# lizhe00/AnimatableGaussians

Hardware: AMD Instinct MI355X
Metric: rendered views/sec (fwd+bwd) @1024^2, ~250k Gaussians (higher is better)
Workload: dtype f32; 1 GPU; BASELINE configs[1]: avatar front|back map, 1 view @1024x1024 per step, rasterizer fwd+bwd through the library-owned step (ag_raster_forward_backward, one native call per view; per-camera argument structures and output images prepared once, FusedRasterStep.prepare / run); gaussians=268348, tiles=4096, views=8, streams=3, prewarm=300, parallelism=1 process

## Files before the change

animatablegaussians_amd/_lib.py:

```python
from __future__ import annotations

import ctypes
import os

import torch

_HERE = os.path.dirname(os.path.abspath(__file__))
LIB_PATH = os.environ.get("AG_LIB_PATH") or os.path.join(_HERE, "lib", "libag_hip.so")

c_i32 = ctypes.c_int32
c_f = ctypes.c_float
c_vp = ctypes.c_void_p
c_sz = ctypes.c_size_t


class AgRasterForwardArgs(ctypes.Structure):
    _fields_ = [
        ("P", c_i32), ("W", c_i32), ("H", c_i32),
        ("sh_degree", c_i32), ("sh_coeffs", c_i32), ("prefiltered", c_i32),
        ("tan_fovx", c_f), ("tan_fovy", c_f), ("scale_modifier", c_f),
        ("bg", c_vp), ("means3D", c_vp), ("colors_precomp", c_vp), ("shs", c_vp), ("opacities", c_vp),
        ("scales", c_vp), ("rotations", c_vp), ("cov3D_precomp", c_vp),
        ("viewmatrix", c_vp), ("projmatrix", c_vp), ("campos", c_vp),
        ("out_color", c_vp), ("out_depth", c_vp), ("out_alpha", c_vp), ("radii", c_vp),
# ... 5 lines not shown

class AgRasterBackwardArgs(ctypes.Structure):
    _fields_ = [
        ("P", c_i32), ("W", c_i32), ("H", c_i32),
        ("sh_degree", c_i32), ("sh_coeffs", c_i32), ("num_rendered", c_i32),
        ("tan_fovx", c_f), ("tan_fovy", c_f), ("scale_modifier", c_f),
        ("bg", c_vp), ("means3D", c_vp), ("radii", c_vp), ("colors_precomp", c_vp), ("shs", c_vp),
        ("scales", c_vp), ("rotations", c_vp), ("cov3D_precomp", c_vp),
        ("viewmatrix", c_vp), ("projmatrix", c_vp), ("campos", c_vp), ("alphas", c_vp),
        ("dL_dout_color", c_vp), ("dL_dout_depth", c_vp), ("dL_dout_alpha", c_vp),
        ("geom_buffer", c_vp), ("image_buffer", c_vp), ("binning_buffer", c_vp),
        ("dL_dmeans2D", c_vp), ("dL_dcolors", c_vp), ("dL_dopacity", c_vp), ("dL_dmeans3D", c_vp),
        ("dL_dcov3D", c_vp), ("dL_dsh", c_vp), ("dL_dscales", c_vp), ("dL_drotations", c_vp),
        ("accum_buffer", c_vp), ("accum_bytes", c_sz), ("accumulate", c_i32), ("reserved", c_i32),
    ]


class AgRasterScratchLayout(ctypes.Structure):
    _fields_ = [(n, c_sz) for n in (
        "geom_rec_off", "geom_rec_stride", "geom_cov3d_off", "geom_tiles_touched_off",
        "img_ranges_off", "img_n_contrib_off", "img_tile_count_off", "img_num_rendered_off",
        "bin_point_list_off", "bin_keys_off")]


class AgGatherArgs(ctypes.Structure):
    _fields_ = [("N", c_i32), ("S", c_i32)] + [(n, c_vp) for n in (
        "pix", "position_map", "other_map", "color_map", "xyz", "opacity_raw", "scaling_raw", "rotation_raw",
        "positions", "opacity", "scales", "rotations", "colors")]


# ... 94 lines not shown
    ("ag_last_error", ctypes.c_char_p, []),
    ("ag_raster_geom_bytes", c_sz, [c_i32]),
    ("ag_raster_image_bytes", c_sz, [c_i32, c_i32]),
    ("ag_raster_binning_bytes", c_sz, [c_i32]),
    ("ag_raster_accum_bytes", c_sz, [c_i32]),
    ("ag_raster_describe_scratch", ctypes.c_int, [c_i32, c_i32, c_i32, c_i32, ctypes.POINTER(AgRasterScratchLayout)]),
    ("ag_raster_forward_plan", ctypes.c_int, [ctypes.POINTER(AgRasterForwardArgs), c_vp, ctypes.POINTER(c_i32)]),
    ("ag_raster_forward_render", ctypes.c_int, [ctypes.POINTER(AgRasterForwardArgs), c_i32, c_vp]),
    ("ag_raster_forward_optimistic", ctypes.c_int, [ctypes.POINTER(AgRasterForwardArgs), c_i32, c_vp, ctypes.POINTER(c_i32)]),
    ("ag_raster_backward", ctypes.c_int, [ctypes.POINTER(AgRasterBackwardArgs), c_vp]),
    ("ag_raster_forward_backward", ctypes.c_int, [ctypes.POINTER(AgRasterForwardArgs), ctypes.POINTER(AgRasterBackwardArgs), c_i32, c_vp,
                                                  ctypes.POINTER(c_i32)]),
    ("ag_raster_forward_backward_enqueue", ctypes.c_int, [ctypes.POINTER(AgRasterForwardArgs), ctypes.POINTER(AgRasterBackwardArgs), c_i32, c_vp,
                                                          ctypes.POINTER(c_i32)]),
    ("ag_raster_collect", ctypes.c_int, [c_i32, ctypes.POINTER(c_i32)]),
    ("ag_raster_large_tile_sort", ctypes.c_int, [c_i32]),
    ("ag_raster_mark_visible", ctypes.c_int, [c_i32, c_vp, c_vp, c_vp, c_vp, c_vp]),
    ("ag_prof_kernel_name", ctypes.c_char_p, [c_i32]),
    ("ag_prof_enable", ctypes.c_int, [ctypes.c_uint32]),
    ("ag_prof_collect", ctypes.c_int, [ctypes.POINTER(c_i32), ctypes.POINTER(c_f), ctypes.POINTER(ctypes.c_double)]),
    ("ag_prof_collect_to", ctypes.c_int, [ctypes.c_char_p, ctypes.POINTER(c_i32), ctypes.POINTER(c_f), ctypes.POINTER(ctypes.c_double)]),
    ("ag_debug_atomic_rate", ctypes.c_int, [c_vp, c_i32, c_i32, c_i32, c_i32, c_vp]),
    ("ag_noise_bias_act_forward", ctypes.c_int, [c_vp, c_vp, c_vp, c_vp, c_vp, ctypes.c_int32, ctypes.c_int32, ctypes.c_float,
                                               ctypes.c_float, c_vp]),
    ("ag_noise_bias_act_partial_floats", c_sz, [c_i32, c_i32]),
    ("ag_noise_bias_act_backward", ctypes.c_int, [c_vp, c_vp, c_vp, c_vp, c_vp, c_vp, c_vp, ctypes.c_int32, ctypes.c_int32,
                                                ctypes.c_float, ctypes.c_float, c_vp]),
    ("ag_modulate_weight_forward", ctypes.c_int, [c_vp, c_vp, c_vp, c_vp, ctypes.c_float, ctypes.c_int32, ctypes.c_int32,
                                                ctypes.c_int32, ctypes.c_int32, ctypes.c_int32, c_vp]),
    ("ag_modulate_weight_partial_floats", c_sz, [c_i32, c_i32]),
# ... 173 lines not shown
```

animatablegaussians_amd/csrc/ag_abi.hip:

```cpp
#include <atomic>
#include <cstdarg>
#include <cstdio>
#include <mutex>
#include <cstring>
#include <vector>

#include "ag_common.h"

namespace ag {

static thread_local char g_err[512] = "";

void set_error(const char* fmt, ...)
{
    va_list ap;
    va_start(ap, fmt);
    vsnprintf(g_err, sizeof(g_err), fmt, ap);
    va_end(ap);
}

int check_hip(hipError_t e, const char* what)
{
    if (e == hipSuccess) return AG_OK;
    set_error("%s: %s", what, hipGetErrorString(e));
// ... 139 lines not shown
    return AG_OK;
}

int ag_raster_forward_optimistic(const AgRasterForwardArgs* a, int32_t capacity, void* stream, int32_t* num_rendered_host)
{
    if (!num_rendered_host) { set_error("null num_rendered_host"); return AG_ERR_INVALID_ARGUMENT; }
    *num_rendered_host = 0;
    if (capacity <= 0) { set_error("capacity must be positive"); return AG_ERR_INVALID_ARGUMENT; }
    int rc = validate_forward(a, true, capacity);
    if (rc) return rc;
    if (a->P == 0) return ag_raster_forward_render(a, 0, stream);
    hipStream_t s = reinterpret_cast<hipStream_t>(stream);
    int32_t* w = pinned_word();
    hipEvent_t ev = plan_event();
    if (!w || !ev) { set_error("hipHostMalloc / hipEventCreate failed"); return AG_ERR_HIP; }
    const bool skip_large = g_large_tiles_seen.load(std::memory_order_relaxed) == 0;
    if ((rc = launch_preprocess(*a, s))) return rc;
    if ((rc = launch_tile_scan(*a, s, (uint32_t)capacity, skip_large))) return rc;
    ImageLayout il((size_t)a->W, (size_t)a->H);
    const char* ib = aligned_base(a->image_buffer);
    if ((rc = check_hip(hipMemcpyAsync(w, ib + il.num_rendered, 4 * sizeof(int32_t), hipMemcpyDeviceToHost, s), "read num_rendered"))) return rc;
    if ((rc = check_hip(hipEventRecord(ev, s), "record plan event"))) return rc;
    if ((rc = launch_bin_sort(*a, capacity, s, skip_large))) return rc;
    if ((rc = launch_blend_forward(*a, capacity, s))) return rc;
    if ((rc = check_hip(hipEventSynchronize(ev), "wait for the instance count"))) return rc;
    *num_rendered_host = w[0];
    if (w[3] > 0) g_large_tiles_seen.store(1, std::memory_order_relaxed);
    if (w[2]) {
        if (w[0] <= capacity) set_error("optimistic forward: %d tiles of >= 2048 instances and the large-class sort was not enqueued for this frame; redo it", w[3]);
        else set_error("optimistic forward: %d instances exceed the capacity of %d; redo with ag_raster_forward_plan + _render", w[0], capacity);
        return AG_ERR_SCRATCH_TOO_SMALL;
    }
    return AG_OK;
}

int ag_raster_forward_render(const AgRasterForwardArgs* a, int32_t R, void* stream)
{
    int rc = validate_forward(a, true, R);
// ... 65 lines not shown
            if (pass == 0 && t.dev != dev) continue;
            if (pass == 1 && t.dev != -1) continue;
            if (t.dev == -1) {
                if (hipHostMalloc(reinterpret_cast<void**>(&t.w), 64, hipHostMallocDefault) != hipSuccess) { t.w = nullptr; return -1; }
                if (hipEventCreateWithFlags(&t.ev, hipEventDisableTiming) != hipSuccess) { (void)hipHostFree(t.w); t.w = nullptr; t.ev = nullptr; return -1; }
                t.dev = dev;
            }
            t.busy = true; t.capacity = capacity;
            return i;
        }
    return -1;
}
}

int ag_raster_forward_backward_enqueue(const AgRasterForwardArgs* f, AgRasterBackwardArgs* b, int32_t capacity, void* stream, int32_t* ticket)
{
    if (!f || !b || !ticket) { set_error("null args"); return AG_ERR_INVALID_ARGUMENT; }
    *ticket = -1;
    if (capacity <= 0) { set_error("capacity must be positive"); return AG_ERR_INVALID_ARGUMENT; }
    if (f->shs && !f->colors_precomp) { set_error("ag_raster_forward_backward: colours-precomp path only"); return AG_ERR_UNSUPPORTED; }
    b->P = f->P; b->W = f->W; b->H = f->H; b->sh_degree = f->sh_degree; b->sh_coeffs = f->sh_coeffs; b->num_rendered = capacity;
    b->tan_fovx = f->tan_fovx; b->tan_fovy = f->tan_fovy; b->scale_modifier = f->scale_modifier;
    b->bg = f->bg; b->means3D = f->means3D; b->radii = f->radii; b->colors_precomp = f->colors_precomp; b->shs = f->shs;
    b->scales = f->scales; b->rotations = f->rotations; b->cov3D_precomp = f->cov3D_precomp;
    b->viewmatrix = f->viewmatrix; b->projmatrix = f->projmatrix; b->campos = f->campos; b->alphas = f->out_alpha;
    b->geom_buffer = f->geom_buffer; b->image_buffer = f->image_buffer; b->binning_buffer = f->binning_buffer;
    int rc = validate_forward(f, true, capacity);
    if (rc) return rc;
    if ((rc = validate_backward(b))) return rc;
    if (f->P == 0) return ag_raster_forward_render(f, 0, stream);
    hipStream_t s = reinterpret_cast<hipStream_t>(stream);
    const int tk = ticket_acquire(capacity);
    if (tk < 0) { set_error("no free read-back ticket (64 views pending) or hipHostMalloc / hipEventCreate failed"); return AG_ERR_HIP; }
    Ticket& t = g_tk[tk];
    auto fail = [&](int code) { std::lock_guard<std::mutex> lk(g_tk_mu); t.busy = false; return code; };
    const bool skip_large = g_large_tiles_seen.load(std::memory_order_relaxed) == 0;
    if ((rc = launch_preprocess(*f, s))) return fail(rc);
    if ((rc = launch_tile_scan(*f, s, (uint32_t)capacity, skip_large))) return fail(rc);
    ImageLayout il((size_t)f->W, (size_t)f->H);
    const char* ib = aligned_base(f->image_buffer);
    if ((rc = check_hip(hipMemcpyAsync(t.w, ib + il.num_rendered, 4 * sizeof(int32_t), hipMemcpyDeviceToHost, s), "read num_rendered"))) return fail(rc);
    if ((rc = check_hip(hipEventRecord(t.ev, s), "record plan event"))) return fail(rc);
    if ((rc = launch_bin_sort(*f, capacity, s, skip_large))) return fail(rc);
    if ((rc = launch_blend_forward(*f, capacity, s))) return fail(rc);
    if ((rc = launch_blend_backward(*b, s))) return fail(rc);
    if ((rc = launch_preprocess_backward(*b, s))) return fail(rc);
    *ticket = tk;
    return AG_OK;
}

int ag_raster_collect(int32_t ticket, int32_t* num_rendered_host)
{
    if (!num_rendered_host) { set_error("null num_rendered_host"); return AG_ERR_INVALID_ARGUMENT; }
    *num_rendered_host = 0;
    if (ticket < 0 || ticket >= kTickets || !g_tk[ticket].busy) { set_error("ag_raster_collect: no such pending view (%d)", ticket); return AG_ERR_INVALID_ARGUMENT; }
    Ticket& t = g_tk[ticket];
    const int rc = check_hip(hipEventSynchronize(t.ev), "wait for the instance count");
    const int32_t n = t.w[0], over = t.w[2], n_large = t.w[3], cap = t.capacity;
    { std::lock_guard<std::mutex> lk(g_tk_mu); t.busy = false; }
    if (rc) return rc;
    *num_rendered_host = n;
    if (n_large > 0) g_large_tiles_seen.store(1, std::memory_order_relaxed);
    if (over) {
        if (n <= cap) set_error("forward+backward: %d tiles of >= 2048 instances and the large-class sort was not enqueued for this view; redo it", n_large);
        else set_error("forward+backward: %d instances exceed the capacity of %d; redo the view with a larger capacity", n, cap);
        return AG_ERR_SCRATCH_TOO_SMALL;
    }
    return AG_OK;
}

int ag_raster_large_tile_sort(int32_t mode)
{
    if (mode == 0 || mode == 1) g_large_tiles_seen.store(mode, std::memory_order_relaxed);
    else if (mode != -1) { set_error("ag_raster_large_tile_sort: mode must be -1 (query), 0 or 1"); return AG_ERR_INVALID_ARGUMENT; }
    return g_large_tiles_seen.load(std::memory_order_relaxed);
}

int ag_raster_forward_backward(const AgRasterForwardArgs* f, AgRasterBackwardArgs* b, int32_t capacity, void* stream,
                               int32_t* num_rendered_host)
// ... 81 lines not shown
```

animatablegaussians_amd/csrc/ag_binning.hip:

```cpp
#include <mutex>

#include "ag_common.h"

namespace ag {

__global__ void __launch_bounds__(1024) tile_scan_kernel(int T, const uint32_t* __restrict__ tile_count,
                                                        uint32_t* __restrict__ cursor, uint2* __restrict__ ranges,
                                                        uint32_t* __restrict__ num_rendered,
                                                        uint4* __restrict__ tile_order, uint32_t capacity, uint32_t skip_large)
{
    __shared__ uint32_t wave_sums[16], wave_ne[16];
    __shared__ uint32_t carry_s, carry_ne;
    __shared__ uint32_t cls_hist[34], cls_off[34];
    const int tid = threadIdx.x, lane = tid & 63, wave = tid >> 6;
    if (tid == 0) { carry_s = 0; carry_ne = 0; }
    if (tid < 34) cls_hist[tid] = 0;
    __syncthreads();
    const uint4* count4 = reinterpret_cast<const uint4*>(tile_count);
    const bool one_pass = T <= 4096;
    uint32_t keep_c[4] = {0u, 0u, 0u, 0u}, keep_st[4] = {0u, 0u, 0u, 0u};
    for (int base = 0; base < T; base += 4096) {
        const int t0 = base + 4 * tid;
        uint32_t c[4] = {0u, 0u, 0u, 0u};
        if (t0 + 3 < T) {
            const uint4 v4 = count4[t0 >> 2];
            c[0] = v4.x; c[1] = v4.y; c[2] = v4.z; c[3] = v4.w;
        } else {
#pragma unroll
            for (int k = 0; k < 4; k++) if (t0 + k < T) c[k] = tile_count[t0 + k];
        }
// ... 21 lines not shown
            r4[0] = make_uint4(c[0] ? start[0] : 0u, c[0] ? start[1] : 0u, c[1] ? start[1] : 0u, c[1] ? start[2] : 0u);
            r4[1] = make_uint4(c[2] ? start[2] : 0u, c[2] ? start[3] : 0u, c[3] ? start[3] : 0u, c[3] ? start[4] : 0u);
        } else {
#pragma unroll
            for (int k = 0; k < 4; k++)
                if (t0 + k < T) {
                    cursor[t0 + k] = start[k];
                    ranges[t0 + k] = c[k] ? make_uint2(start[k], start[k + 1]) : make_uint2(0u, 0u);
                }
        }
#pragma unroll
        for (int k = 0; k < 4; k++)
            if (t0 + k < T) {
                if (c[k]) {
                    atomicAdd(&cls_hist[32 - __clz(c[k])], 1u);
                    ne_before++;
                } else {
                    tile_order[(uint32_t)(T - 1) - ((uint32_t)(t0 + k) - ne_before)] = make_uint4((uint32_t)(t0 + k), 0u, 0u, 0u);
                }
            }
#pragma unroll
        for (int k = 0; k < 4; k++) { keep_c[k] = c[k]; keep_st[k] = start[k]; }
        __syncthreads();
        if (tid == 1023) { carry_s = start[4]; carry_ne = ne_before; }
        __syncthreads();
    }
    if (tid == 0) {
        uint32_t n_large = 0;
        for (int cls = 12; cls < 34; cls++) n_large += cls_hist[cls];
        const bool over = carry_s > capacity || (skip_large && n_large > 0u);
        num_rendered[0] = carry_s;
        num_rendered[1] = over ? 0u : carry_ne;
        num_rendered[2] = over ? 1u : 0u;
        num_rendered[3] = n_large;
    }
    if (tid == 0) {
        uint32_t acc = 0;
        for (int cls = 33; cls >= 1; cls--) { cls_off[cls] = acc; acc += cls_hist[cls]; }
    }
    __syncthreads();
    for (int base = 0; base < T; base += 4096) {
        const int t0 = base + 4 * tid;
        if (t0 >= T) break;
        uint32_t c[4] = {0u, 0u, 0u, 0u}, st[4] = {0u, 0u, 0u, 0u};
        if (one_pass) {
#pragma unroll
            for (int k = 0; k < 4; k++) { c[k] = keep_c[k]; st[k] = keep_st[k]; }
        } else if (t0 + 3 < T) {
            const uint4 v4 = count4[t0 >> 2], s4 = reinterpret_cast<const uint4*>(cursor)[t0 >> 2];
            c[0] = v4.x; c[1] = v4.y; c[2] = v4.z; c[3] = v4.w;
            st[0] = s4.x; st[1] = s4.y; st[2] = s4.z; st[3] = s4.w;
        } else {
#pragma unroll
            for (int k = 0; k < 4; k++) if (t0 + k < T) { c[k] = tile_count[t0 + k]; st[k] = cursor[t0 + k]; }
        }
#pragma unroll
        for (int k = 0; k < 4; k++)
            if (t0 + k < T) {
                if (c[k]) tile_order[atomicAdd(&cls_off[32 - __clz(c[k])], 1u)] = make_uint4((uint32_t)(t0 + k), st[k], st[k] + c[k], 0u);
            }
    }
}

int launch_tile_scan(const AgRasterForwardArgs& a, hipStream_t s, uint32_t capacity, bool skip_large)
{
    const int gx = (a.W + kTileX - 1) / kTileX, gy = (a.H + kTileY - 1) / kTileY;
    char* ib = aligned_base(a.image_buffer);
    ImageLayout il((size_t)a.W, (size_t)a.H);
    { ProfScope ps(AG_K_TILE_SCAN, s); hipLaunchKernelGGL(tile_scan_kernel, dim3(1), dim3(1024), 0, s, gx * gy,
                       reinterpret_cast<const uint32_t*>(ib + il.tile_count),
                       reinterpret_cast<uint32_t*>(ib + il.cursor),
                       reinterpret_cast<uint2*>(ib + il.ranges),
                       reinterpret_cast<uint32_t*>(ib + il.num_rendered),
                       reinterpret_cast<uint4*>(ib + il.tile_order), capacity, skip_large ? 1u : 0u); }
    return check_hip(hipGetLastError(), "tile_scan_kernel");
}

__device__ __forceinline__ void get_rect_i(float px, float py, int max_radius, int gx, int gy,
                                           uint32_t& x0o, uint32_t& y0o, uint32_t& x1o, uint32_t& y1o)
{
    const float r = (float)max_radius;
    int x0 = (int)((px - r) / (float)kTileX);
    int y0 = (int)((py - r) / (float)kTileY);
    int x1 = (int)((px + r + (float)kTileX - 1.0f) / (float)kTileX);
    int y1 = (int)((py + r + (float)kTileY - 1.0f) / (float)kTileY);
    x0 = max(0, x0); y0 = max(0, y0); x1 = max(0, x1); y1 = max(0, y1);
    x0o = (uint32_t)min(gx, x0); y0o = (uint32_t)min(gy, y0);
    x1o = (uint32_t)min(gx, x1); y1o = (uint32_t)min(gy, y1);
}
// ... 153 lines not shown
            const uint32_t blk = t >> lk, off = t & (hk - 1);
            const uint32_t i = (blk << (lk + 1)) + off, p = (blk << (lk + 1)) + k - 1 - off;
            if (p < n) { const uint64_t a = sk[i], b = sk[p]; if (a > b) { sk[i] = b; sk[p] = a; } }
        }
        __syncthreads();
        for (uint32_t j = k >> 2; j > 0; j >>= 1) {
            for (uint32_t t = tid; t < half; t += nthreads) {
                const uint32_t i = ((t & ~(j - 1)) << 1) | (t & (j - 1)), p = i + j;
                if (p < n) { const uint64_t a = sk[i], b = sk[p]; if (a > b) { sk[i] = b; sk[p] = a; } }
            }
            __syncthreads();
        }
    }
}

template <int NT, int KPT, bool PRESORTED>
__device__ __forceinline__ void sort_segment_lds(uint64_t* __restrict__ sk, const uint64_t* __restrict__ seg, uint32_t n, uint32_t run0,
                                                 uint32_t* __restrict__ out_list, uint64_t* __restrict__ out_keys, int tid)
{
    constexpr uint32_t CAP = NT * KPT;
    uint64_t* bufA = sk;
    uint64_t* bufB = sk + CAP;
    uint64_t v[KPT];
    const uint32_t base = (uint32_t)tid * (uint32_t)KPT;
#pragma unroll
    for (int i = 0; i < KPT; i++) v[i] = (base + i < n) ? seg[base + i] : kKeyInf;
    constexpr bool WAVE_RUNS = !PRESORTED && KPT == 4 && AG_SORT_WAVE_NETWORK;
    if constexpr (WAVE_RUNS) {
        if constexpr (KPT == 4) wave_sort256(v, tid & 63);
    } else if (!PRESORTED) sort_regs<KPT>(v);
    if (base < n) {
#pragma unroll
        for (int i = 0; i < KPT; i++) bufA[base + i] = v[i];
    }
    __syncthreads();
    const uint32_t n8 = (n + (uint32_t)KPT - 1u) & ~((uint32_t)KPT - 1u);
    for (uint32_t L = PRESORTED ? run0 : (WAVE_RUNS ? 256u : (uint32_t)KPT); L < n8; L <<= 1) {
        if (base < n8) {
            const uint32_t ps = base & ~(2u * L - 1u);
            const uint32_t o = base - ps;
            const uint32_t lx = min(L, n8 - ps);
            const uint32_t ly = (ps + L < n8) ? min(L, n8 - ps - L) : 0u;
            const uint64_t* X = bufA + ps;
            const uint64_t* Y = bufA + ps + L;
            uint32_t lo = (o > ly) ? o - ly : 0u, hi = min(o, lx);
            while (lo < hi) {
                const uint32_t mid = (lo + hi) >> 1;
                if (X[mid] < Y[o - mid - 1]) lo = mid + 1; else hi = mid;
            }
            uint32_t i = lo, j = o - lo;
            uint64_t xv = (i < lx) ? X[i] : kKeyInf, yv = (j < ly) ? Y[j] : kKeyInf;
#pragma unroll
            for (int r = 0; r < KPT; r++) {
                const bool takex = xv <= yv;
                bufB[base + r] = takex ? xv : yv;
                if (takex) { i++; xv = (i < lx) ? X[i] : kKeyInf; }
                else       { j++; yv = (j < ly) ? Y[j] : kKeyInf; }
            }
        }
        __syncthreads();
        uint64_t* t = bufA; bufA = bufB; bufB = t;
    }
    if (out_list) { for (uint32_t i = tid; i < n; i += NT) out_list[i] = (uint32_t)bufA[i]; }
    else          { for (uint32_t i = tid; i < n; i += NT) out_keys[i] = bufA[i]; }
}

template <int NT, bool LARGE, int KPT>
__global__ void __launch_bounds__(NT) tile_sort_kernel(const uint4* __restrict__ tile_order, const uint32_t* __restrict__ counts,
                                                      uint64_t* __restrict__ keys, uint32_t* __restrict__ point_list)
{
    extern __shared__ __attribute__((aligned(16))) uint64_t sk[];
    constexpr uint32_t CAP = NT * KPT;
    const uint32_t n_active = counts[1];
    const int tid = threadIdx.x;
    if (!LARGE) {
        for (uint32_t item = gridDim.x - 1u - blockIdx.x; item < 4u * n_active; item += gridDim.x) {
            const uint4 wd = tile_order[item >> 2];
            const uint32_t n = wd.z - wd.y;
            if (n < 2048u) break;
            if (n <= (uint32_t)kSortSmallCap || n > (uint32_t)kSortLargeCap) continue;
            const uint32_t c0 = (item & 3u) * (uint32_t)kSortSmallCap;
            if (c0 >= n) continue;
            __syncthreads();
            uint64_t* seg = keys + wd.y + c0;
            sort_segment_lds<NT, KPT, false>(sk, seg, min((uint32_t)kSortSmallCap, n - c0), 0u, nullptr, seg, tid);
        }
    }
    for (uint32_t rank = blockIdx.x; rank < n_active; rank += gridDim.x) {
    const uint4 wd = tile_order[rank];
    const uint2 rg = make_uint2(wd.y, wd.z);
    const uint32_t n = rg.y - rg.x;
    if (LARGE) { if (n < 2048u) break; if (n <= (uint32_t)kSortSmallCap) continue; }
    else if (n > (uint32_t)kSortSmallCap) continue;
    uint64_t* seg = keys + rg.x;
    __syncthreads();
    if (n > CAP) {
        uint32_t m = 2;
        while (m < n) m <<= 1;
        bitonic_sort_global(seg, n, m, tid, NT);
        for (uint32_t i = tid; i < n; i += NT) point_list[rg.x + i] = (uint32_t)seg[i];
        continue;
    }
    if (LARGE) sort_segment_lds<NT, KPT, true>(sk, seg, n, (uint32_t)kSortSmallCap, point_list + rg.x, nullptr, tid);
    else       sort_segment_lds<NT, KPT, false>(sk, seg, n, 0u, point_list + rg.x, nullptr, tid);
    }
}

int launch_bin_sort(const AgRasterForwardArgs& a, int R, hipStream_t s, bool skip_large)
{
    const int gx = (a.W + kTileX - 1) / kTileX, gy = (a.H + kTileY - 1) / kTileY;
    if (R <= 0) return AG_OK;
    char* gb = aligned_base(a.geom_buffer);
    char* ib = aligned_base(a.image_buffer);
    char* bb = aligned_base(a.binning_buffer);
    GeomLayout gl((size_t)a.P);
    ImageLayout il((size_t)a.W, (size_t)a.H);
    BinLayout bl((size_t)R);
    uint64_t* keys = reinterpret_cast<uint64_t*>(bb + bl.keys);
    uint32_t* point_list = reinterpret_cast<uint32_t*>(bb + bl.point_list);
    { ProfScope ps(AG_K_SCATTER, s); hipLaunchKernelGGL(scatter_kernel, dim3((a.P + 255) / 256), dim3(256), 0, s, a.P, gx, gy, a.radii,
                       reinterpret_cast<const GaussRec*>(gb + gl.rec), reinterpret_cast<uint32_t*>(ib + il.cursor), keys,
                       reinterpret_cast<const uint32_t*>(ib + il.num_rendered)); }
    if (check_hip(hipGetLastError(), "scatter_kernel")) return AG_ERR_HIP;
// ... 4 lines not shown
        int dev = 0;
        (void)hipGetDevice(&dev);
        std::lock_guard<std::mutex> lk(mu);
        if (dev < 0 || dev >= 64 || !((done >> dev) & 1)) {
            if (check_hip(hipFuncSetAttribute(reinterpret_cast<const void*>(&tile_sort_kernel<1024, true, 8>),
                                              hipFuncAttributeMaxDynamicSharedMemorySize, (int)kLargeLds), "sort LDS attr"))
                return AG_ERR_HIP;
            if (dev >= 0 && dev < 64) done |= 1ull << dev;
        }
    }
    {
        ProfScope ps(AG_K_TILE_SORT, s);
        const uint4* order = reinterpret_cast<const uint4*>(ib + il.tile_order);
        const uint32_t* counts = reinterpret_cast<const uint32_t*>(ib + il.num_rendered);
        const int T = gx * gy;
        hipLaunchKernelGGL((tile_sort_kernel<512, false, 4>), dim3(T < 1280 ? T : 1280), dim3(512), kSmallLds, s, order, counts, keys, point_list);
        if (!skip_large)
            hipLaunchKernelGGL((tile_sort_kernel<1024, true, 8>), dim3(T < 256 ? T : 256), dim3(1024), kLargeLds, s, order, counts, keys, point_list);
    }
    return check_hip(hipGetLastError(), "tile_sort_kernel");
}

}
```

animatablegaussians_amd/csrc/ag_common.h:

```cpp
#pragma once

#include <hip/hip_runtime.h>
#include <stddef.h>
#include <stdint.h>

#include "../../include/ag_raster.h"

namespace ag {

constexpr int kTileX = AG_TILE_X;
constexpr int kTileY = AG_TILE_Y;
constexpr int kWave = 64;

struct __attribute__((aligned(16))) GaussRec {
    float x, y;
    float ca, cb;
    float cc, op;
    float r, g;
    float b, depth;
    float r2cut;
    float qcut;
};
static_assert(sizeof(GaussRec) == 48, "GaussRec must be 48 bytes");

// ... 68 lines not shown
        clamped = o;        o = align_up(o + P * 3, 256);
        total = o + 256;
    }
};

struct ImageLayout {
    size_t ranges, tile_count, cursor, n_contrib, num_rendered, tile_order, total;
    __host__ __device__ ImageLayout(size_t W, size_t H)
    {
        const size_t T = ((W + kTileX - 1) / kTileX) * ((H + kTileY - 1) / kTileY);
        size_t o = 0;
        ranges = o;        o = align_up(o + T * 2 * sizeof(uint32_t), 256);
        tile_count = o;    o = align_up(o + T * sizeof(uint32_t), 256);
        cursor = o;        o = align_up(o + T * sizeof(uint32_t), 256);
        n_contrib = o;     o = align_up(o + W * H * sizeof(uint32_t), 256);
        num_rendered = o;  o = align_up(o + 16, 256);
        tile_order = o;    o = align_up(o + T * 4 * sizeof(uint32_t), 256);
        total = o + 256;
    }
};

struct BinLayout {
    size_t keys, point_list, total;
    __host__ __device__ explicit BinLayout(size_t R)
    {
        size_t o = 0;
        keys = o;        o = align_up(o + R * sizeof(uint64_t), 256);
        point_list = o;  o = align_up(o + R * sizeof(uint32_t), 256);
        total = o + 256;
    }
};
// ... 5 lines not shown

void set_error(const char* fmt, ...);

int prof_begin(int kernel_id, hipStream_t s, double work, const char* tag = nullptr);
void prof_end(int handle, hipStream_t s);
struct ProfScope {
    int handle; hipStream_t s;
    ProfScope(int id, hipStream_t s_, double work = 0.0, const char* tag = nullptr) : handle(prof_begin(id, s_, work, tag)), s(s_) {}
    ~ProfScope() { prof_end(handle, s); }
    ProfScope(const ProfScope&) = delete;
    ProfScope& operator=(const ProfScope&) = delete;
};
int check_hip(hipError_t e, const char* what);

int launch_preprocess(const AgRasterForwardArgs& a, hipStream_t s);
int launch_tile_scan(const AgRasterForwardArgs& a, hipStream_t s, uint32_t capacity = 0xffffffffu, bool skip_large = false);
int launch_bin_sort(const AgRasterForwardArgs& a, int R, hipStream_t s, bool skip_large = false);
int launch_blend_forward(const AgRasterForwardArgs& a, int R, hipStream_t s);
int launch_blend_backward(const AgRasterBackwardArgs& a, hipStream_t s);
int launch_preprocess_backward(const AgRasterBackwardArgs& a, hipStream_t s);
int launch_debug_atomic_rate(float* accum, int lines, int blocks, int iters, int comps, hipStream_t s);
int launch_mark_visible(int P, const float* means3D, const float* view, uint8_t* present, hipStream_t s);

}
```

animatablegaussians_amd/rasterizer.py:

```python
from __future__ import annotations

import ctypes
from typing import NamedTuple, Optional, Tuple

import torch
import torch.nn as nn

from . import _lib

NUM_CHANNELS = 3


def _ptr(t: Optional[torch.Tensor]):
    if t is None or t.numel() == 0:
        return None
    return ctypes.c_void_p(t.data_ptr())


def _f32c(t: torch.Tensor, name: str) -> torch.Tensor:
    if t.dtype is torch.float32 and t.is_cuda and t.is_contiguous():
        return t
    if t.numel() == 0:
        return t
    if not t.is_cuda:
# ... 254 lines not shown
            raise Exception('Please provide excatly one of either SHs or precomputed colors!')
        has_sr = scales is not None or rotations is not None
        if ((scales is None or rotations is None) and cov3D_precomp is None) or (has_sr and cov3D_precomp is not None):
            raise Exception('Please provide exactly one of either scale/rotation pair or precomputed 3D covariance!')
        empty = torch.Tensor([])
        shs = empty if shs is None else shs
        colors_precomp = empty if colors_precomp is None else colors_precomp
        scales = empty if scales is None else scales
        rotations = empty if rotations is None else rotations
        cov3D_precomp = empty if cov3D_precomp is None else cov3D_precomp
        return rasterize_gaussians(means3D, means2D, shs, colors_precomp, opacities, scales, rotations, cov3D_precomp,
                                   self.raster_settings)


class _PreparedView:
    __slots__ = ("a", "b", "slot", "color", "depth", "alpha", "radii", "keep", "inputs", "in_ptrs", "checked", "image_grads")


class FusedRasterStep:

    _GRADS = (("dL_dmeans2D", 3), ("dL_dcolors", 3), ("dL_dopacity", 1), ("dL_dmeans3D", 3), ("dL_dcov3D", 6), ("dL_dscales", 3),
              ("dL_drotations", 4))

    def __init__(self, P: int, W: int, H: int, device, n_streams: int = 2):
        self.P, self.W, self.H = int(P), int(W), int(H)
        self.dev = torch.device(device)
        if self.dev.index is None:
            self.dev = torch.device("cuda", torch.cuda.current_device())
        self.key = (self.P, self.W, self.H, self.dev.index)
        byte = dict(dtype=torch.uint8, device=self.dev)
        self.slots = []
# ... 30 lines not shown
        a.P, a.W, a.H = P, W, H
        a.sh_degree = a.sh_coeffs = 0
        a.prefiltered = int(bool(rs.prefiltered))
        a.tan_fovx, a.tan_fovy, a.scale_modifier = float(rs.tanfovx), float(rs.tanfovy), float(rs.scale_modifier)
        a.bg, a.viewmatrix, a.projmatrix, a.campos = (_ptr(t) for t in cam)
        a.out_color = _ptr(h.color); a.out_depth = _ptr(h.depth); a.out_alpha = _ptr(h.alpha); a.radii = _ptr(h.radii)
        a.geom_buffer = _ptr(sl["geom"]); a.geom_bytes = sl["geom"].numel()
        a.image_buffer = _ptr(sl["img"]); a.image_bytes = sl["img"].numel()
        b = h.b = _lib.AgRasterBackwardArgs()
        g = sl["grads"]
        b.dL_dmeans2D = _ptr(g["dL_dmeans2D"]); b.dL_dcolors = _ptr(g["dL_dcolors"]); b.dL_dopacity = _ptr(g["dL_dopacity"])
        b.dL_dmeans3D = _ptr(g["dL_dmeans3D"]); b.dL_dcov3D = _ptr(g["dL_dcov3D"]); b.dL_dscales = _ptr(g["dL_dscales"])
        b.dL_drotations = _ptr(g["dL_drotations"])
        b.accum_buffer = _ptr(sl["accum"]); b.accum_bytes = sl["accum"].numel()
        h.inputs = h.in_ptrs = None
        self._set_image_grads(h, g_color, g_depth, g_alpha)
        return h

    @staticmethod
    def _set_image_grads(h, g_color, g_depth, g_alpha):
        gs = [_f32c(t, n) for t, n in ((g_color, "dL_dout_color"), (g_depth, "dL_dout_depth"), (g_alpha, "dL_dout_alpha"))]
        h.image_grads = gs
        h.b.dL_dout_color, h.b.dL_dout_depth, h.b.dL_dout_alpha = (_ptr(t) for t in gs)

    def run(self, h: "_PreparedView", means3D, colors, opacities, scales, rotations, image_grads=None, accumulate: bool = False,
            inputs_outlive_join: bool = False):
        L = _lib.lib()
        P, dev = self.P, self.dev
        sl = self.slots[h.slot]
        self._collect(sl)
# ... 4 lines not shown
            chk = [_f32c(t, n) for t, n in zip(ins, ("means3D", "colors_precomp", "opacities", "scales", "rotations"))]
            a = h.a
            a.means3D, a.colors_precomp, a.opacities, a.scales, a.rotations = (_ptr(t) for t in chk)
            h.inputs, h.in_ptrs, h.checked = ins, [t.data_ptr() for t in ins], chk
        if image_grads is not None:
            self._set_image_grads(h, *image_grads)
        a, b = h.a, h.b
        b.accumulate = int(bool(accumulate and sl["used"]))
        st = sl["stream"]
        st.wait_stream(torch.cuda.current_stream(dev))
        with _on_device(dev):
            cap = _capacity.get(self.key) or (4 * P + 4096)
            binning = self._binning(sl, cap)
            a.binning_buffer = binning.data_ptr(); a.binning_bytes = binning.numel()
            tk = ctypes.c_int32(-1)
            _lib.check(L.ag_raster_forward_backward_enqueue(ctypes.byref(a), ctypes.byref(b), cap, ctypes.c_void_p(st.cuda_stream), ctypes.byref(tk)),
                       "ag_raster_forward_backward_enqueue")
        if tk.value >= 0:
            sl["pending"] = (tk.value, h, cap)
            if not _capacity.get(self.key):
                self._collect(sl)
        sl["used"] = True
        if not inputs_outlive_join:
            for t in h.checked + h.image_grads:
                t.record_stream(st)
        return h.color, h.depth, h.alpha, h.radii, sl["grads"]

    def _collect(self, sl):
        pend = sl.get("pending")
        if pend is None:
            return
        sl["pending"] = None
        tk, h, cap = pend
        L = _lib.lib()
        R = ctypes.c_int32(0)
        with _on_device(self.dev):
            rc = L.ag_raster_collect(tk, ctypes.byref(R))
            while rc == _lib.AG_ERR_SCRATCH_TOO_SMALL:
                cap = int(R.value) + int(R.value) // 4 + 1024
                binning = self._binning(sl, cap)
                h.a.binning_buffer = binning.data_ptr(); h.a.binning_bytes = binning.numel()
                rc = L.ag_raster_forward_backward(ctypes.byref(h.a), ctypes.byref(h.b), cap, ctypes.c_void_p(sl["stream"].cuda_stream), ctypes.byref(R))
            _lib.check(rc, "ag_raster_forward_backward")
        want = int(R.value) + int(R.value) // 4 + 1024
        if want > _capacity.get(self.key, 0):
            _capacity[self.key] = want

    def view(self, rs: GaussianRasterizationSettings, means3D, colors, opacities, scales, rotations, g_color, g_depth, g_alpha,
             accumulate: bool = False, slot: Optional[int] = None):
        P, W, H, dev = self.P, self.W, self.H, self.dev
        if int(means3D.size(0)) != P or int(rs.image_width) != W or int(rs.image_height) != H:
            raise RuntimeError("FusedRasterStep: sizes differ from the ones it was built for")
# ... 43 lines not shown
```

include/ag_raster.h:

```cpp
#ifndef AG_RASTER_H
#define AG_RASTER_H

#include <stddef.h>
#include <stdint.h>

#ifdef __cplusplus
extern "C" {
#endif

#define AG_ABI_VERSION 1

#define AG_OK 0
#define AG_ERR_INVALID_ARGUMENT (-1)
#define AG_ERR_SCRATCH_TOO_SMALL (-2)
#define AG_ERR_HIP (-3)
#define AG_ERR_UNSUPPORTED (-4)
#define AG_ERR_RANGE (-5)

#define AG_TILE_X 16
#define AG_TILE_Y 16

typedef struct AgRasterForwardArgs {
    int32_t P;
    int32_t W, H;
// ... 83 lines not shown
int ag_raster_forward_plan(const AgRasterForwardArgs* args, void* stream, int32_t* num_rendered_host);

int ag_raster_forward_render(const AgRasterForwardArgs* args, int32_t num_rendered, void* stream);

int ag_raster_forward_optimistic(const AgRasterForwardArgs* args, int32_t capacity, void* stream, int32_t* num_rendered_host);

int ag_raster_backward(const AgRasterBackwardArgs* args, void* stream);

int ag_raster_forward_backward(const AgRasterForwardArgs* fwd, AgRasterBackwardArgs* bwd, int32_t capacity, void* stream,
                               int32_t* num_rendered_host);

int ag_raster_forward_backward_enqueue(const AgRasterForwardArgs* fwd, AgRasterBackwardArgs* bwd, int32_t capacity, void* stream,
                                       int32_t* ticket);
int ag_raster_collect(int32_t ticket, int32_t* num_rendered_host);

int ag_raster_mark_visible(int32_t P, const float* means3D, const float* viewmatrix, const float* projmatrix,
                           uint8_t* present, void* stream);

enum AgKernelId {
    AG_K_PREPROCESS = 0,
    AG_K_TILE_SCAN = 1,
    AG_K_SCATTER = 2,
    AG_K_TILE_SORT = 3,
    AG_K_BLEND_FORWARD = 4,
    AG_K_BLEND_BACKWARD = 5,
    AG_K_PREPROCESS_BACKWARD = 6,
    AG_K_GATHER_CONV = 7,
    AG_K_WGRAD = 8,
    AG_K_COUNT = 9
};
// ... 14 lines not shown
```

Baseline: 7312 views/s.

## Size large-tile sort launch from per-camera hints of large-tile counts

```diff
diff --git a/animatablegaussians_amd/_lib.py b/animatablegaussians_amd/_lib.py
--- a/animatablegaussians_amd/_lib.py
+++ b/animatablegaussians_amd/_lib.py
@@ -43,6 +43,10 @@
         ("dL_dcov3D", c_vp), ("dL_dsh", c_vp), ("dL_dscales", c_vp), ("dL_drotations", c_vp),
         ("accum_buffer", c_vp), ("accum_bytes", c_sz), ("accumulate", c_i32), ("reserved", c_i32),
     ]
+
+
+class AgRasterSortHint(ctypes.Structure):
+    _fields_ = [("large_tiles", c_i32), ("longest_tile", c_i32)]
 
 
 class AgRasterScratchLayout(ctypes.Structure):
@@ -167,6 +171,9 @@
     ("ag_raster_forward_backward_enqueue", ctypes.c_int, [ctypes.POINTER(AgRasterForwardArgs), ctypes.POINTER(AgRasterBackwardArgs), c_i32, c_vp,
                                                           ctypes.POINTER(c_i32)]),
     ("ag_raster_collect", ctypes.c_int, [c_i32, ctypes.POINTER(c_i32)]),
+    ("ag_raster_forward_backward_enqueue_hinted", ctypes.c_int, [ctypes.POINTER(AgRasterForwardArgs), ctypes.POINTER(AgRasterBackwardArgs), c_i32,
+                                                                 ctypes.POINTER(AgRasterSortHint), c_vp, ctypes.POINTER(c_i32)]),
+    ("ag_raster_collect_counts", ctypes.c_int, [c_i32, ctypes.POINTER(c_i32), ctypes.POINTER(AgRasterSortHint)]),
     ("ag_raster_large_tile_sort", ctypes.c_int, [c_i32]),
     ("ag_raster_mark_visible", ctypes.c_int, [c_i32, c_vp, c_vp, c_vp, c_vp, c_vp]),
     ("ag_prof_kernel_name", ctypes.c_char_p, [c_i32]),
diff --git a/animatablegaussians_amd/csrc/ag_abi.hip b/animatablegaussians_amd/csrc/ag_abi.hip
--- a/animatablegaussians_amd/csrc/ag_abi.hip
+++ b/animatablegaussians_amd/csrc/ag_abi.hip
@@ -177,14 +177,14 @@
     int32_t* w = pinned_word();
     hipEvent_t ev = plan_event();
     if (!w || !ev) { set_error("hipHostMalloc / hipEventCreate failed"); return AG_ERR_HIP; }
-    const bool skip_large = g_large_tiles_seen.load(std::memory_order_relaxed) == 0;
+    const LargeSortPlan large = g_large_tiles_seen.load(std::memory_order_relaxed) == 0 ? LargeSortPlan::none() : LargeSortPlan();
     if ((rc = launch_preprocess(*a, s))) return rc;
-    if ((rc = launch_tile_scan(*a, s, (uint32_t)capacity, skip_large))) return rc;
+    if ((rc = launch_tile_scan(*a, s, (uint32_t)capacity, large.longest_allowed()))) return rc;
     ImageLayout il((size_t)a->W, (size_t)a->H);
     const char* ib = aligned_base(a->image_buffer);
     if ((rc = check_hip(hipMemcpyAsync(w, ib + il.num_rendered, 4 * sizeof(int32_t), hipMemcpyDeviceToHost, s), "read num_rendered"))) return rc;
     if ((rc = check_hip(hipEventRecord(ev, s), "record plan event"))) return rc;
-    if ((rc = launch_bin_sort(*a, capacity, s, skip_large))) return rc;
+    if ((rc = launch_bin_sort(*a, capacity, s, large))) return rc;
     if ((rc = launch_blend_forward(*a, capacity, s))) return rc;
     if ((rc = check_hip(hipEventSynchronize(ev), "wait for the instance count"))) return rc;
     *num_rendered_host = w[0];
@@ -280,6 +280,12 @@
 }
 
 int ag_raster_forward_backward_enqueue(const AgRasterForwardArgs* f, AgRasterBackwardArgs* b, int32_t capacity, void* stream, int32_t* ticket)
+{
+    return ag_raster_forward_backward_enqueue_hinted(f, b, capacity, nullptr, stream, ticket);
+}
+
+int ag_raster_forward_backward_enqueue_hinted(const AgRasterForwardArgs* f, AgRasterBackwardArgs* b, int32_t capacity, const AgRasterSortHint* expected,
+                                              void* stream, int32_t* ticket)
 {
     if (!f || !b || !ticket) { set_error("null args"); return AG_ERR_INVALID_ARGUMENT; }
     *ticket = -1;
@@ -300,14 +306,15 @@
     if (tk < 0) { set_error("no free read-back ticket (64 views pending) or hipHostMalloc / hipEventCreate failed"); return AG_ERR_HIP; }
     Ticket& t = g_tk[tk];
     auto fail = [&](int code) { std::lock_guard<std::mutex> lk(g_tk_mu); t.busy = false; return code; };
-    const bool skip_large = g_large_tiles_seen.load(std::memory_order_relaxed) == 0;
+    const LargeSortPlan large = (expected && expected->large_tiles >= 0) ? large_sort_plan(expected->large_tiles, expected->longest_tile)
+                                : g_large_tiles_seen.load(std::memory_order_relaxed) == 0 ? LargeSortPlan::none() : LargeSortPlan();
     if ((rc = launch_preprocess(*f, s))) return fail(rc);
-    if ((rc = launch_tile_scan(*f, s, (uint32_t)capacity, skip_large))) return fail(rc);
+    if ((rc = launch_tile_scan(*f, s, (uint32_t)capacity, large.longest_allowed()))) return fail(rc);
     ImageLayout il((size_t)f->W, (size_t)f->H);
     const char* ib = aligned_base(f->image_buffer);
-    if ((rc = check_hip(hipMemcpyAsync(t.w, ib + il.num_rendered, 4 * sizeof(int32_t), hipMemcpyDeviceToHost, s), "read num_rendered"))) return fail(rc);
+    if ((rc = check_hip(hipMemcpyAsync(t.w, ib + il.num_rendered, 5 * sizeof(int32_t), hipMemcpyDeviceToHost, s), "read num_rendered"))) return fail(rc);
     if ((rc = check_hip(hipEventRecord(t.ev, s), "record plan event"))) return fail(rc);
-    if ((rc = launch_bin_sort(*f, capacity, s, skip_large))) return fail(rc);
+    if ((rc = launch_bin_sort(*f, capacity, s, large))) return fail(rc);
     if ((rc = launch_blend_forward(*f, capacity, s))) return fail(rc);
     if ((rc = launch_blend_backward(*b, s))) return fail(rc);
     if ((rc = launch_preprocess_backward(*b, s))) return fail(rc);
@@ -315,20 +322,24 @@
     return AG_OK;
 }
 
-int ag_raster_collect(int32_t ticket, int32_t* num_rendered_host)
-{
+int ag_raster_collect(int32_t ticket, int32_t* num_rendered_host) { return ag_raster_collect_counts(ticket, num_rendered_host, nullptr); }
+
+int ag_raster_collect_counts(int32_t ticket, int32_t* num_rendered_host, AgRasterSortHint* seen)
+{
+    if (seen) { seen->large_tiles = -1; seen->longest_tile = 0; }
     if (!num_rendered_host) { set_error("null num_rendered_host"); return AG_ERR_INVALID_ARGUMENT; }
     *num_rendered_host = 0;
     if (ticket < 0 || ticket >= kTickets || !g_tk[ticket].busy) { set_error("ag_raster_collect: no such pending view (%d)", ticket); return AG_ERR_INVALID_ARGUMENT; }
     Ticket& t = g_tk[ticket];
     const int rc = check_hip(hipEventSynchronize(t.ev), "wait for the instance count");
-    const int32_t n = t.w[0], over = t.w[2], n_large = t.w[3], cap = t.capacity;
+    const int32_t n = t.w[0], over = t.w[2], n_large = t.w[3], longest = t.w[4], cap = t.capacity;
     { std::lock_guard<std::mutex> lk(g_tk_mu); t.busy = false; }
     if (rc) return rc;
     *num_rendered_host = n;
+    if (seen) { seen->large_tiles = n_large; seen->longest_tile = longest; }
     if (n_large > 0) g_large_tiles_seen.store(1, std::memory_order_relaxed);
     if (over) {
-        if (n <= cap) set_error("forward+backward: %d tiles of >= 2048 instances and the large-class sort was not enqueued for this view; redo it", n_large);
+        if (n <= cap) set_error("forward+backward: %d tiles of >= 2048 instances (the longest %d) and the large-class sort enqueued for this view does not take them; redo it", n_large, longest);
         else set_error("forward+backward: %d instances exceed the capacity of %d; redo the view with a larger capacity", n, cap);
         return AG_ERR_SCRATCH_TOO_SMALL;
     }
diff --git a/animatablegaussians_amd/csrc/ag_binning.hip b/animatablegaussians_amd/csrc/ag_binning.hip
--- a/animatablegaussians_amd/csrc/ag_binning.hip
+++ b/animatablegaussians_amd/csrc/ag_binning.hip
@@ -7,13 +7,14 @@
 __global__ void __launch_bounds__(1024) tile_scan_kernel(int T, const uint32_t* __restrict__ tile_count,
                                                         uint32_t* __restrict__ cursor, uint2* __restrict__ ranges,
                                                         uint32_t* __restrict__ num_rendered,
-                                                        uint4* __restrict__ tile_order, uint32_t capacity, uint32_t skip_large)
+                                                        uint4* __restrict__ tile_order, uint32_t capacity, uint32_t large_allowed)
 {
     __shared__ uint32_t wave_sums[16], wave_ne[16];
     __shared__ uint32_t carry_s, carry_ne;
     __shared__ uint32_t cls_hist[34], cls_off[34];
+    __shared__ uint32_t longest_large;
     const int tid = threadIdx.x, lane = tid & 63, wave = tid >> 6;
-    if (tid == 0) { carry_s = 0; carry_ne = 0; }
+    if (tid == 0) { carry_s = 0; carry_ne = 0; longest_large = 0; }
     if (tid < 34) cls_hist[tid] = 0;
     __syncthreads();
     const uint4* count4 = reinterpret_cast<const uint4*>(tile_count);
@@ -65,6 +66,7 @@
             if (t0 + k < T) {
                 if (c[k]) {
                     atomicAdd(&cls_hist[32 - __clz(c[k])], 1u);
+                    if (c[k] >= 2048u) atomicMax(&longest_large, c[k]);
                     ne_before++;
                 } else {
                     tile_order[(uint32_t)(T - 1) - ((uint32_t)(t0 + k) - ne_before)] = make_uint4((uint32_t)(t0 + k), 0u, 0u, 0u);
@@ -79,11 +81,12 @@
     if (tid == 0) {
         uint32_t n_large = 0;
         for (int cls = 12; cls < 34; cls++) n_large += cls_hist[cls];
-        const bool over = carry_s > capacity || (skip_large && n_large > 0u);
+        const bool over = carry_s > capacity || (n_large > 0u && longest_large > large_allowed);
         num_rendered[0] = carry_s;
         num_rendered[1] = over ? 0u : carry_ne;
         num_rendered[2] = over ? 1u : 0u;
         num_rendered[3] = n_large;
+        num_rendered[4] = longest_large;
     }
     if (tid == 0) {
         uint32_t acc = 0;
@@ -113,7 +116,7 @@
     }
 }
 
-int launch_tile_scan(const AgRasterForwardArgs& a, hipStream_t s, uint32_t capacity, bool skip_large)
+int launch_tile_scan(const AgRasterForwardArgs& a, hipStream_t s, uint32_t capacity, uint32_t large_allowed)
 {
     const int gx = (a.W + kTileX - 1) / kTileX, gy = (a.H + kTileY - 1) / kTileY;
     char* ib = aligned_base(a.image_buffer);
@@ -123,7 +126,7 @@
                        reinterpret_cast<uint32_t*>(ib + il.cursor),
                        reinterpret_cast<uint2*>(ib + il.ranges),
                        reinterpret_cast<uint32_t*>(ib + il.num_rendered),
-                       reinterpret_cast<uint4*>(ib + il.tile_order), capacity, skip_large ? 1u : 0u); }
+                       reinterpret_cast<uint4*>(ib + il.tile_order), capacity, large_allowed); }
     return check_hip(hipGetLastError(), "tile_scan_kernel");
 }
 
@@ -307,13 +310,12 @@
     }
 }
 
-template <int NT, int KPT, bool PRESORTED>
-__device__ __forceinline__ void sort_segment_lds(uint64_t* __restrict__ sk, const uint64_t* __restrict__ seg, uint32_t n, uint32_t run0,
-                                                 uint32_t* __restrict__ out_list, uint64_t* __restrict__ out_keys, int tid)
-{
-    constexpr uint32_t CAP = NT * KPT;
+template <int NT, int KPT, bool PRESORTED, bool DIRECT>
+__device__ __forceinline__ void sort_segment_lds(uint64_t* __restrict__ sk, uint32_t bufb_off, const uint64_t* __restrict__ seg, uint32_t n,
+                                                 uint32_t run0, uint32_t* __restrict__ out_list, uint64_t* __restrict__ out_keys, int tid)
+{
     uint64_t* bufA = sk;
-    uint64_t* bufB = sk + CAP;
+    uint64_t* bufB = sk + bufb_off;
     uint64_t v[KPT];
     const uint32_t base = (uint32_t)tid * (uint32_t)KPT;
 #pragma unroll
@@ -329,6 +331,7 @@
     __syncthreads();
     const uint32_t n8 = (n + (uint32_t)KPT - 1u) & ~((uint32_t)KPT - 1u);
     for (uint32_t L = PRESORTED ? run0 : (WAVE_RUNS ? 256u : (uint32_t)KPT); L < n8; L <<= 1) {
+        const bool last = DIRECT && (L << 1) >= n8;
         if (base < n8) {
             const uint32_t ps = base & ~(2u * L - 1u);
             const uint32_t o = base - ps;
@@ -346,11 +349,14 @@
 #pragma unroll
             for (int r = 0; r < KPT; r++) {
                 const bool takex = xv <= yv;
-                bufB[base + r] = takex ? xv : yv;
+                const uint64_t ov = takex ? xv : yv;
+                if (!last) bufB[base + r] = ov;
+                else if (base + r < n) { if (out_list) out_list[base + r] = (uint32_t)ov; else out_keys[base + r] = ov; }
                 if (takex) { i++; xv = (i < lx) ? X[i] : kKeyInf; }
                 else       { j++; yv = (j < ly) ? Y[j] : kKeyInf; }
             }
         }
+        if (last) return;
         __syncthreads();
         uint64_t* t = bufA; bufA = bufB; bufB = t;
     }
@@ -360,7 +366,7 @@
 
 template <int NT, bool LARGE, int KPT>
 __global__ void __launch_bounds__(NT) tile_sort_kernel(const uint4* __restrict__ tile_order, const uint32_t* __restrict__ counts,
-                                                      uint64_t* __restrict__ keys, uint32_t* __restrict__ point_list)
+                                                      uint64_t* __restrict__ keys, uint32_t* __restrict__ point_list, uint32_t lds_keys)
 {
     extern __shared__ __attribute__((aligned(16))) uint64_t sk[];
     constexpr uint32_t CAP = NT * KPT;
@@ -376,7 +382,7 @@
             if (c0 >= n) continue;
             __syncthreads();
             uint64_t* seg = keys + wd.y + c0;
-            sort_segment_lds<NT, KPT, false>(sk, seg, min((uint32_t)kSortSmallCap, n - c0), 0u, nullptr, seg, tid);
+            sort_segment_lds<NT, KPT, false, false>(sk, CAP, seg, min((uint32_t)kSortSmallCap, n - c0), 0u, nullptr, seg, tid);
         }
     }
     for (uint32_t rank = blockIdx.x; rank < n_active; rank += gridDim.x) {
@@ -394,12 +400,29 @@
         for (uint32_t i = tid; i < n; i += NT) point_list[rg.x + i] = (uint32_t)seg[i];
         continue;
     }
-    if (LARGE) sort_segment_lds<NT, KPT, true>(sk, seg, n, (uint32_t)kSortSmallCap, point_list + rg.x, nullptr, tid);
-    else       sort_segment_lds<NT, KPT, false>(sk, seg, n, 0u, point_list + rg.x, nullptr, tid);
-    }
-}
-
-int launch_bin_sort(const AgRasterForwardArgs& a, int R, hipStream_t s, bool skip_large)
+    if (LARGE) {
+        if (n > lds_keys) continue;
+        sort_segment_lds<NT, KPT, true, true>(sk, lds_keys, seg, n, (uint32_t)kSortSmallCap, point_list + rg.x, nullptr, tid);
+    } else sort_segment_lds<NT, KPT, false, false>(sk, CAP, seg, n, 0u, point_list + rg.x, nullptr, tid);
+    }
+}
+
+LargeSortPlan large_sort_plan(int expected_tiles, int expected_longest)
+{
+    LargeSortPlan p;
+    if (expected_tiles < 0) return p;
+    if (expected_tiles == 0) return LargeSortPlan::none();
+    const uint32_t n = (uint32_t)expected_tiles;
+    p.grid = n + n / 4u < 256u ? n + n / 4u : 256u;
+    if (expected_longest > 0 && expected_longest <= kSortLargeCap) {
+        const uint32_t m = (uint32_t)expected_longest + (uint32_t)expected_longest / 8u;
+        const uint32_t k = (m + 1023u) & ~1023u;
+        p.lds_keys = k < (uint32_t)kSortLargeCap ? k : (uint32_t)kSortLargeCap;
+    }
+    return p;
+}
+
+int launch_bin_sort(const AgRasterForwardArgs& a, int R, hipStream_t s, LargeSortPlan large)
 {
     const int gx = (a.W + kTileX - 1) / kTileX, gy = (a.H + kTileY - 1) / kTileY;
     if (R <= 0) return AG_OK;
@@ -434,9 +457,13 @@
         const uint4* order = reinterpret_cast<const uint4*>(ib + il.tile_order);
         const uint32_t* counts = reinterpret_cast<const uint32_t*>(ib + il.num_rendered);
         const int T = gx * gy;
-        hipLaunchKernelGGL((tile_sort_kernel<512, false, 4>), dim3(T < 1280 ? T : 1280), dim3(512), kSmallLds, s, order, counts, keys, point_list);
-        if (!skip_large)
-            hipLaunchKernelGGL((tile_sort_kernel<1024, true, 8>), dim3(T < 256 ? T : 256), dim3(1024), kLargeLds, s, order, counts, keys, point_list);
+        hipLaunchKernelGGL((tile_sort_kernel<512, false, 4>), dim3(T < 1280 ? T : 1280), dim3(512), kSmallLds, s, order, counts, keys, point_list, 0u);
+        if (large.grid > 0) {
+            const uint32_t lk = large.lds_keys < (uint32_t)kSortLargeCap ? large.lds_keys : (uint32_t)kSortLargeCap;
+            const size_t lds = (lk <= 2u * kSortSmallCap ? 1ull : 2ull) * lk * sizeof(uint64_t);
+            const int grid = (int)large.grid < T ? (int)large.grid : T;
+            hipLaunchKernelGGL((tile_sort_kernel<1024, true, 8>), dim3(grid), dim3(1024), lds, s, order, counts, keys, point_list, lk);
+        }
     }
     return check_hip(hipGetLastError(), "tile_sort_kernel");
 }
diff --git a/animatablegaussians_amd/csrc/ag_common.h b/animatablegaussians_amd/csrc/ag_common.h
--- a/animatablegaussians_amd/csrc/ag_common.h
+++ b/animatablegaussians_amd/csrc/ag_common.h
@@ -106,7 +106,7 @@
         tile_count = o;    o = align_up(o + T * sizeof(uint32_t), 256);
         cursor = o;        o = align_up(o + T * sizeof(uint32_t), 256);
         n_contrib = o;     o = align_up(o + W * H * sizeof(uint32_t), 256);
-        num_rendered = o;  o = align_up(o + 16, 256);
+        num_rendered = o;  o = align_up(o + 32, 256);
         tile_order = o;    o = align_up(o + T * 4 * sizeof(uint32_t), 256);
         total = o + 256;
     }
@@ -142,8 +142,15 @@
 int check_hip(hipError_t e, const char* what);
 
 int launch_preprocess(const AgRasterForwardArgs& a, hipStream_t s);
-int launch_tile_scan(const AgRasterForwardArgs& a, hipStream_t s, uint32_t capacity = 0xffffffffu, bool skip_large = false);
-int launch_bin_sort(const AgRasterForwardArgs& a, int R, hipStream_t s, bool skip_large = false);
+constexpr uint32_t kLargeSortAny = 0xffffffffu;
+struct LargeSortPlan {
+    uint32_t grid = 256, lds_keys = 8192;
+    static LargeSortPlan none() { LargeSortPlan p; p.grid = 0; return p; }
+    uint32_t longest_allowed() const { return grid == 0 ? 0u : (lds_keys >= 8192u ? kLargeSortAny : lds_keys); }
+};
+LargeSortPlan large_sort_plan(int expected_tiles, int expected_longest);
+int launch_tile_scan(const AgRasterForwardArgs& a, hipStream_t s, uint32_t capacity = 0xffffffffu, uint32_t large_allowed = kLargeSortAny);
+int launch_bin_sort(const AgRasterForwardArgs& a, int R, hipStream_t s, LargeSortPlan large = LargeSortPlan());
 int launch_blend_forward(const AgRasterForwardArgs& a, int R, hipStream_t s);
 int launch_blend_backward(const AgRasterBackwardArgs& a, hipStream_t s);
 int launch_preprocess_backward(const AgRasterBackwardArgs& a, hipStream_t s);
diff --git a/animatablegaussians_amd/rasterizer.py b/animatablegaussians_amd/rasterizer.py
--- a/animatablegaussians_amd/rasterizer.py
+++ b/animatablegaussians_amd/rasterizer.py
@@ -292,7 +292,8 @@
 
 
 class _PreparedView:
-    __slots__ = ("a", "b", "slot", "color", "depth", "alpha", "radii", "keep", "inputs", "in_ptrs", "checked", "image_grads")
+    __slots__ = ("a", "b", "slot", "color", "depth", "alpha", "radii", "keep", "inputs", "in_ptrs", "checked", "image_grads", "sort_hint",
+                 "sort_seen")
 
 
 class FusedRasterStep:
@@ -353,6 +354,8 @@
         b.dL_drotations = _ptr(g["dL_drotations"])
         b.accum_buffer = _ptr(sl["accum"]); b.accum_bytes = sl["accum"].numel()
         h.inputs = h.in_ptrs = None
+        h.sort_hint = _lib.AgRasterSortHint(-1, 0)
+        h.sort_seen = _lib.AgRasterSortHint(-1, 0)
         self._set_image_grads(h, g_color, g_depth, g_alpha)
         return h
 
@@ -387,8 +390,9 @@
             binning = self._binning(sl, cap)
             a.binning_buffer = binning.data_ptr(); a.binning_bytes = binning.numel()
             tk = ctypes.c_int32(-1)
-            _lib.check(L.ag_raster_forward_backward_enqueue(ctypes.byref(a), ctypes.byref(b), cap, ctypes.c_void_p(st.cuda_stream), ctypes.byref(tk)),
-                       "ag_raster_forward_backward_enqueue")
+            _lib.check(L.ag_raster_forward_backward_enqueue_hinted(ctypes.byref(a), ctypes.byref(b), cap, ctypes.byref(h.sort_hint),
+                                                                   ctypes.c_void_p(st.cuda_stream), ctypes.byref(tk)),
+                       "ag_raster_forward_backward_enqueue_hinted")
         if tk.value >= 0:
             sl["pending"] = (tk.value, h, cap)
             if not _capacity.get(self.key):
@@ -408,7 +412,9 @@
         L = _lib.lib()
         R = ctypes.c_int32(0)
         with _on_device(self.dev):
-            rc = L.ag_raster_collect(tk, ctypes.byref(R))
+            rc = L.ag_raster_collect_counts(tk, ctypes.byref(R), ctypes.byref(h.sort_seen))
+            if h.sort_seen.large_tiles >= 0:
+                h.sort_hint.large_tiles, h.sort_hint.longest_tile = h.sort_seen.large_tiles, h.sort_seen.longest_tile
             while rc == _lib.AG_ERR_SCRATCH_TOO_SMALL:
                 cap = int(R.value) + int(R.value) // 4 + 1024
                 binning = self._binning(sl, cap)
diff --git a/include/ag_raster.h b/include/ag_raster.h
--- a/include/ag_raster.h
+++ b/include/ag_raster.h
@@ -121,6 +121,14 @@
                                        int32_t* ticket);
 int ag_raster_collect(int32_t ticket, int32_t* num_rendered_host);
 
+typedef struct AgRasterSortHint {
+    int32_t large_tiles;
+    int32_t longest_tile;
+} AgRasterSortHint;
+int ag_raster_forward_backward_enqueue_hinted(const AgRasterForwardArgs* fwd, AgRasterBackwardArgs* bwd, int32_t capacity,
+                                              const AgRasterSortHint* expected, void* stream, int32_t* ticket);
+int ag_raster_collect_counts(int32_t ticket, int32_t* num_rendered_host, AgRasterSortHint* seen);
+
 int ag_raster_mark_visible(int32_t P, const float* means3D, const float* viewmatrix, const float* projmatrix,
                            uint8_t* present, void* stream);
 
diff --git a/profiles/large_tile_counts.py b/profiles/large_tile_counts.py
--- /dev/null
+++ b/profiles/large_tile_counts.py
@@ -0,0 +1,19 @@
+import os
+import sys
+
+import numpy as np
+
+ROOT = os.path.dirname(os.path.dirname(os.path.abspath(__file__)))
+sys.path.insert(0, ROOT)
+sys.path.insert(0, os.path.join(ROOT, "tests"))
+import helpers as h
+from animatablegaussians_amd import synth
+
+av = synth.avatar_map_gaussians()
+print("camera,instances,non_empty_tiles,tiles_ge_2048,tiles_2049_4096,tiles_4097_8192,tiles_gt_8192,longest,tiles_1024_2047")
+for vi, camd in enumerate(synth.free_view_cameras(8, img=1024)):
+    scene = dict(av, **camd)
+    fw = h.gpu_native_forward(scene, h.cam_of(scene))
+    n = (fw["ranges"][:, 1].astype(np.int64) - fw["ranges"][:, 0]).astype(np.int64)
+    print(f"{vi},{fw['num_rendered']},{int((n > 0).sum())},{int((n >= 2048).sum())},{int(((n > 2048) & (n <= 4096)).sum())},"
+          f"{int(((n > 4096) & (n <= 8192)).sum())},{int((n > 8192).sum())},{int(n.max())},{int(((n >= 1024) & (n < 2048)).sum())}", flush=True)
diff --git a/profiles/tile_sort_trace.py b/profiles/tile_sort_trace.py
--- /dev/null
+++ b/profiles/tile_sort_trace.py
@@ -0,0 +1,86 @@
+import collections
+import sqlite3
+import statistics
+import sys
+
+
+def load(path):
+    db = sqlite3.connect(path)
+    cur = db.execute("select * from kernels")
+    cols = [c[0] for c in cur.description]
+    lane = next((c for c in ("stream_id", "queue_id", "stream", "queue") if c in cols), None)
+    if lane is None:
+        raise SystemExit(f"no stream / queue column in the kernels view: {cols}")
+    i_name, i_s, i_e, i_l = cols.index("name"), cols.index("start"), cols.index("end"), cols.index(lane)
+    rows = [(r[i_l], r[i_s], r[i_e], r[i_name]) for r in cur]
+    return lane, rows
+
+
+def main():
+    path = sys.argv[1]
+    steps = int(sys.argv[2]) if len(sys.argv) > 2 else 2000
+    warmup = int(sys.argv[3]) if len(sys.argv) > 3 else 200
+    ncam = int(sys.argv[4]) if len(sys.argv) > 4 else 8
+    lane, rows = load(path)
+    per = collections.defaultdict(list)
+    for ln, s, e, name in rows:
+        if any(k in name for k in ("preprocess_kernel", "scatter_kernel", "tile_sort_kernel", "tile_scan_kernel", "blend_")):
+            per[ln].append((s, e, name))
+    views = {}
+    for ln, ks in per.items():
+        ks.sort()
+        cur = None
+        out = []
+        for k in ks:
+            if "preprocess_kernel" in k[2] and "backward" not in k[2]:
+                cur = [k]
+                out.append(cur)
+            elif cur is not None:
+                cur.append(k)
+        views[ln] = out
+    lanes = sorted((ln for ln in views if len(views[ln]) > steps // 8), key=lambda ln: views[ln][-1][0][0], reverse=True)
+    n_l = len(lanes)
+    print(f"# {path}: lanes by {lane}: {[(ln, len(views[ln])) for ln in lanes]}")
+    last = warmup + steps - 1
+    stat = collections.defaultdict(lambda: collections.defaultdict(list))
+    for j, ln in enumerate(lanes):
+        vs = views[ln]
+        for back in range(len(vs)):
+            step = last - j - back * n_l
+            if step < warmup:
+                break
+            v = vs[len(vs) - 1 - back]
+            cam = step % ncam
+            sc = [k for k in v if "scatter_kernel" in k[2]]
+            small = [k for k in v if "tile_sort_kernel" in k[2] and "false" in k[2]]
+            large = [k for k in v if "tile_sort_kernel" in k[2] and "true" in k[2]]
+            st = stat[cam]
+            st["views"].append(1)
+            if sc and small:
+                st["small_us"].append((small[0][1] - small[0][0]) / 1e3)
+                st["gap_small_us"].append((small[0][0] - sc[0][1]) / 1e3)
+            if small and large:
+                st["large_us"].append((large[0][1] - large[0][0]) / 1e3)
+                st["gap_large_us"].append((large[0][0] - small[0][1]) / 1e3)
+            if sc:
+                nxt = [k for k in v if k[0] > sc[0][0] and "blend_forward" in k[2]]
+                if nxt:
+                    st["scatter_end_to_blend_start_us"].append((nxt[0][0] - sc[0][1]) / 1e3)
+    med = lambda a: statistics.median(a) if a else float("nan")
+    print("camera,views,large_launches,small_med_us,small_p90_us,gap_scatter_to_small_med_us,large_med_us,large_p90_us,large_min_us,"
+          "gap_small_to_large_med_us,scatter_end_to_blend_start_med_us")
+    tot = collections.defaultdict(list)
+    for cam in sorted(stat):
+        st = stat[cam]
+        p90 = lambda a: sorted(a)[int(0.9 * (len(a) - 1))] if a else float("nan")
+        print(f"{cam},{len(st['views'])},{len(st['large_us'])},{med(st['small_us']):.2f},{p90(st['small_us']):.2f},{med(st['gap_small_us']):.2f},"
+              f"{med(st['large_us']):.2f},{p90(st['large_us']):.2f},{min(st['large_us'], default=float('nan')):.2f},{med(st['gap_large_us']):.2f},"
+              f"{med(st['scatter_end_to_blend_start_us']):.2f}")
+        for k, a in st.items():
+            tot[k] += a
+    print(f"all,{len(tot['views'])},{len(tot['large_us'])},{med(tot['small_us']):.2f},,{med(tot['gap_small_us']):.2f},{med(tot['large_us']):.2f},,"
+          f"{min(tot['large_us'], default=float('nan')):.2f},{med(tot['gap_large_us']):.2f},{med(tot['scatter_end_to_blend_start_us']):.2f}")
+
+
+if __name__ == "__main__":
+    main()
```

After: 7236 views/s. -1.0%, worse.
